# MuMuJun97/semantic_slam_mapping

Hardware: AMD Instinct MI355X
Metric: frames/sec semantic-mapping, 640x480 RGB-D (higher is better)
Workload: dtype u8; 1 GPU; configs[1]: synthetic 640x480 RGB-D + precomputed 12-class masks, 1k frames per GPU, ORB 1000 kp/frame, 5 ref frames, leaf 0.10 m; frames_per_gpu=1000, frames_all_gpus=1000, batch_frames=250, matcher_halo_frames=0, parallelism=single GPU

## Files before the change

semantic_slam_mapping_amd/csrc/kernels_orb.hip:

```cpp
#include "ssm_internal.h"
#include "../../include/ssm/fast_quick_core.h"
#include <cstdlib>
#include <type_traits>
#include <algorithm>
#include <cstring>
#include <vector>

#define WAVE 64

template <bool VEC>
__global__ void gray_kernel(const uint8_t* __restrict__ img, int W, int H, int stride0, uint8_t* __restrict__ pyr, int pyr_bytes)
{
    const int quads = stride0 >> 2;
    const int q = blockIdx.x * blockDim.x + threadIdx.x;
    if (q >= quads * H) return;
    const int y = q / quads, x = (q - y * quads) << 2;
    const uint8_t* src = img + (size_t)blockIdx.y * W * H * 3 + ((size_t)y * W + x) * 3;
    uint8_t* dst = pyr + (size_t)blockIdx.y * pyr_bytes + (size_t)y * stride0 + x;
    uint32_t out = 0;
    if (x >= W) { *reinterpret_cast<uint32_t*>(dst) = 0; return; }
    if (VEC) {
        const uint32_t* s = reinterpret_cast<const uint32_t*>(src);
        uint32_t a = s[0], b = s[1], c = s[2];
        uint32_t p0 = ((a & 255) * 1868 + ((a >> 8) & 255) * 9617 + ((a >> 16) & 255) * 4899 + 8192) >> 14;
// ... 858 lines not shown
    for (int k = 0; k < OT_T / 64; k++) { const uint32_t x = sw[k]; tot += x; if (k < w) base += x; }
    __syncthreads();
    total = tot;
    return inc - v + base;
}
#ifdef SSM_OT_PROF
__device__ unsigned long long ot_prof[8][8];
#define OTP_T0 long long otp_ = clock64();
#define OTP(k) { const long long n_ = clock64(); if (threadIdx.x == 0) atomicAdd(&ot_prof[blockIdx.y & 7][k], (unsigned long long)(n_ - otp_)); otp_ = n_; }
#define OTP_CNT(k) { if (threadIdx.x == 0) atomicAdd(&ot_prof[blockIdx.y & 7][k], 1ull); }
#else
#define OTP_T0
#define OTP(k)
#define OTP_CNT(k)
#endif
template <int NODES>
__global__ void __launch_bounds__(OT_T, NODES == 256 ? 8 : 1)
octree_kernel(OrbGeom g, const cand_t* __restrict__ cand, const int32_t* __restrict__ ncand, const int32_t* __restrict__ cellmax,
              uint16_t* __restrict__ node_of, uint32_t* __restrict__ sel, int32_t* __restrict__ nsel, int32_t* __restrict__ status)
{
    __shared__ QNode    nd[2][NODES];
    __shared__ uint32_t cnt[2][NODES];
    __shared__ uint32_t sq[2][NODES];
    __shared__ __attribute__((aligned(8))) uint32_t cc[NODES][4];
    __shared__ short    newpos[NODES];
    __shared__ __attribute__((aligned(8))) short childpos[NODES][4];
    __shared__ short    order[NODES];
    unsigned long long* best = reinterpret_cast<unsigned long long*>(&cc[0][0]);
    __shared__ uint16_t lnof[OT_KCAP];
    __shared__ uint16_t cumn[NODES];
    __shared__ uint32_t sscan[OT_T / 64];
    __shared__ int sL, sFinish, sMode, sErr, sValid, sFirst;
    const int l = blockIdx.y, f = blockIdx.x, tid = threadIdx.x;
    OTP_T0
    const LevelGeom& L = g.L[l];
    const int N = L.nfeat;
    int nc = ncand[f * g.nlevels + l];
    if (nc > L.cand_cap) { nc = L.cand_cap; if (tid == 0) atomicOr(status, 1); }
    const cand_t* gkeys = cand + (size_t)f * g.cand_total + L.cand_off;
    uint16_t* gnof = node_of + (size_t)f * g.cand_total + L.cand_off;
    const bool in_lds = nc <= OT_KCAP;
    constexpr int KPT = OT_KCAP / OT_T;
    uint32_t kxr[KPT];
#pragma unroll
    for (int u = 0; u < KPT; u++) kxr[u] = 0u;
#define KEY(i) (gkeys[i])
#define KEYX(i) (gkeys[i].x)
#define NOF(i) (in_lds ? lnof[i] : gnof[i])
#define SETNOF(i, v) do { if (in_lds) lnof[i] = (uint16_t)(v); else gnof[i] = (uint16_t)(v); } while (0)
    uint32_t* out = sel + (size_t)f * g.sel_total + L.sel_off;
    if (nc == 0) { if (tid == 0) nsel[f * g.nlevels + l] = 0; return; }
    const int nIni = L.nIni; const float hX = L.hX;
    for (int i = tid; i < nIni; i += OT_T) {
        QNode q; q.x0 = (short)(int)(hX * (float)i); q.y0 = 0; q.x1 = (short)(int)(hX * (float)(i + 1)); q.y1 = (short)(L.maxBY - L.minBY);
        nd[0][i] = q; cnt[0][i] = 0; sq[0][i] = i;
    }
    if (tid == 0) { sErr = 0; sValid = 0; }
    __syncthreads();
    const int32_t* cm = cellmax + (size_t)f * g.cells_total + L.cell_off;
    int nvalid = 0;
    auto init_trip = [&](auto lds_tag, int i0, cand_t (&k)[OT_UN]) {
        constexpr bool in_lds = decltype(lds_tag)::value;
        int cmv[OT_UN];
#pragma unroll
        for (int u = 0; u < OT_UN; u++) { const int i = i0 + u * OT_T; k[u] = i < nc ? KEY(i) : make_uint2(0u, 0u); }
#pragma unroll
// ... 9 lines not shown
            int b = (int)((float)x / hX); b = min(b, nIni - 1);
            SETNOF(i, b); atomicAdd(&cnt[0][b], 1u); nvalid++;
        }
    };
    if (in_lds) {
#pragma unroll
        for (int t = 0; t < KPT / OT_UN; t++) {
            const int i0 = tid + t * OT_UN * OT_T;
            if (i0 < nc) { cand_t k[OT_UN]; init_trip(std::true_type{}, i0, k); for (int u = 0; u < OT_UN; u++) kxr[t * OT_UN + u] = k[u].x; }
        }
    } else {
        for (int i0 = tid; i0 < nc; i0 += OT_UN * OT_T) { cand_t k[OT_UN]; init_trip(std::false_type{}, i0, k); }
    }
    if (nvalid) atomicAdd(&sValid, nvalid);
    __syncthreads();
    if (sValid == 0) { if (tid == 0) nsel[f * g.nlevels + l] = 0; return; }
    if (tid == 0) {
        int pos = 0;
        for (int i = 0; i < nIni; i++) {
            if (cnt[0][i] == 0) { newpos[i] = -1; continue; }
            nd[1][pos] = nd[0][i]; cnt[1][pos] = cnt[0][i]; sq[1][pos] = sq[0][i]; newpos[i] = (short)pos; pos++;
        }
        sL = pos; sFinish = 0; sMode = 0;
    }
    __syncthreads();
    if (in_lds) { for (int i = tid; i < nc; i += OT_T) { const int o = lnof[i]; if (o != DROPPED) lnof[i] = (uint16_t)newpos[o]; } }
    else        { for (int i = tid; i < nc; i += OT_T) { const int o = gnof[i]; if (o != DROPPED) gnof[i] = (uint16_t)newpos[o]; } }
    int cur = 1;
    __syncthreads();
    OTP(0)
    while (!sFinish) {
// ... 205 lines not shown
    if (sErr && tid == 0) atomicOr(status, 2);
    for (int i = tid; i < Lf; i += OT_T) best[i] = 0ull;
    __syncthreads();
    for (int i0 = tid; i0 < nc; i0 += OT_UN * OT_T) {
        int ni[OT_UN]; cand_t k[OT_UN];
#pragma unroll
        for (int u = 0; u < OT_UN; u++) { const int i = i0 + u * OT_T; ni[u] = i < nc ? (in_lds ? (int)lnof[i] : (int)gnof[i]) : DROPPED; k[u] = i < nc ? KEY(i) : make_uint2(0u, 0u); }
#pragma unroll
        for (int u = 0; u < OT_UN; u++) {
            if (ni[u] == DROPPED) continue;
            const unsigned long long v = ((unsigned long long)(k[u].x >> 24) << 56) | ((unsigned long long)(0xFFFFFFFFu - k[u].y) << 24) | (k[u].x & 0xFFFFFFu);
            atomicMax(&best[ni[u]], v);
        }
    }
    __syncthreads();
    for (int i = tid; i < Lf && i < L.sel_cap; i += OT_T) {
        const unsigned long long v = best[i];
        const uint32_t x = (uint32_t)(v & 4095) + L.minBX, y = (uint32_t)((v >> 12) & 4095) + L.minBY, s = (uint32_t)(v >> 56);
        out[i] = x | (y << 12) | (s << 24);
    }
    if (tid == 0) { nsel[f * g.nlevels + l] = min(Lf, L.sel_cap); if (Lf > L.sel_cap) atomicOr(status, 4); }
    OTP(5)
}
#ifdef SSM_OT_PROF
extern "C" void ssm_debug_octree_prof(void)
{
    unsigned long long h[8][8];
    if (hipMemcpyFromSymbol(h, HIP_SYMBOL(ot_prof), sizeof(h)) != hipSuccess) return;
    for (int l = 0; l < 8; l++) fprintf(stderr, "octree level %d: init %llu count-sweep %llu order %llu rebuild %llu relabel %llu best %llu | passes %llu\n", l, h[l][0], h[l][1], h[l][2], h[l][3], h[l][4], h[l][5], h[l][7]);
    for (auto& r_ : h) for (auto& v_ : r_) v_ = 0;
    (void)hipMemcpyToSymbol(HIP_SYMBOL(ot_prof), h, sizeof(h));
}
#endif
hipError_t k_octree(int n, const OrbGeom& g, const cand_t* cand, const int32_t* ncand, const int32_t* cellmax, uint16_t* node_of,
                    uint32_t* sel, int32_t* nsel, int32_t* status, hipStream_t s)
{
    int need = 0;
    for (int l = 0; l < g.nlevels; l++) need = need > g.L[l].nfeat + 3 ? need : g.L[l].nfeat + 3;
    for (int l = 0; l < g.nlevels; l++) need = need > 4 * g.L[l].nIni + 8 ? need : 4 * g.L[l].nIni + 8;
    if (need <= 256 - 8) octree_kernel<256><<<dim3(n, g.nlevels), OT_T, 0, s>>>(g, cand, ncand, cellmax, node_of, sel, nsel, status);
    else if (need <= 512 - 8) octree_kernel<512><<<dim3(n, g.nlevels), OT_T, 0, s>>>(g, cand, ncand, cellmax, node_of, sel, nsel, status);
    else                 octree_kernel<1024><<<dim3(n, g.nlevels), OT_T, 0, s>>>(g, cand, ncand, cellmax, node_of, sel, nsel, status);
    return hipGetLastError();
}

__device__ __forceinline__ float fast_atan2_deg(float y, float x)
{
    const float p1 = 0.9997878412794807f * (float)(180 / 3.14159265358979323846);
    const float p3 = -0.3258083974640975f * (float)(180 / 3.14159265358979323846);
    const float p5 = 0.1555786518463281f * (float)(180 / 3.14159265358979323846);
    const float p7 = -0.04432655554792128f * (float)(180 / 3.14159265358979323846);
    const float ax = fabsf(x), ay = fabsf(y);
    float a, c, c2;
    if (ax >= ay) { c = ay / (ax + (float)2.2204460492503131e-16); c2 = c * c; a = (((p7 * c2 + p5) * c2 + p3) * c2 + p1) * c; }
    else          { c = ax / (ay + (float)2.2204460492503131e-16); c2 = c * c; a = 90.f - (((p7 * c2 + p5) * c2 + p3) * c2 + p1) * c; }
    if (x < 0) a = 180.f - a;
    if (y < 0) a = 360.f - a;
// ... 17 lines not shown
    const double sn = r + r * (r2 * ps);
    double pc = 1.0 / 20922789888000.0;
    pc = pc * r2 - 1.0 / 87178291200.0;
    pc = pc * r2 + 1.0 / 479001600.0;
    pc = pc * r2 - 1.0 / 3628800.0;
    pc = pc * r2 + 1.0 / 40320.0;
    pc = pc * r2 - 1.0 / 720.0;
    pc = pc * r2 + 1.0 / 24.0;
    pc = pc * r2 - 0.5;
    const double cs = 1.0 + r2 * pc;
    double S, C;
    switch (k & 3) { case 0: S = sn; C = cs; break; case 1: S = cs; C = -sn; break; case 2: S = -sn; C = -cs; break; default: S = -cs; C = sn; break; }
    *s = (float)S; *c = (float)C;
}
__device__ __forceinline__ int wave_total(int v) { return __builtin_amdgcn_readlane((int)wave_incl_scan_u32((uint32_t)v), 63); }
struct KpAux { int32_t m10, m01; float sn, cs; };
#define DP_ROWS_O 31
#define DP_QW_O 3
#define DP_ROWS_B 37
#define DP_QW_B 4
__device__ __forceinline__ bool kp_slot(const OrbGeom& g, const int32_t* __restrict__ ns, int slot, int& l, int& oidx)
{
    if (slot >= g.sel_total) return false;
    l = 0;
    while (l + 1 < g.nlevels && slot >= g.L[l+1].sel_off) l++;
    const int i = slot - g.L[l].sel_off;
    if (i >= ns[l]) return false;
    oidx = i;
    for (int k = 0; k < l; k++) oidx += ns[k];
    return true;
}
struct KpRec { uint32_t off; uint32_t stride_level; int32_t oidx; uint32_t pk; };
__global__ void __launch_bounds__(256)
kp_prepare_kernel(OrbGeom g, const uint32_t* __restrict__ sel, const int32_t* __restrict__ nsel, KpRec* __restrict__ recs, int32_t* __restrict__ nkp)
{
    const int f = blockIdx.y, slot = blockIdx.x * 256 + threadIdx.x;
    const int32_t* ns = nsel + f * g.nlevels;
    if (slot == 0) { int t = 0; for (int l = 0; l < g.nlevels; l++) t += ns[l]; nkp[f] = t; }
    if (slot >= g.sel_total) return;
    int l, oidx;
    KpRec r; r.off = 0; r.stride_level = 0; r.oidx = -1; r.pk = 0;
    if (kp_slot(g, ns, slot, l, oidx)) {
        const LevelGeom& L = g.L[l];
        r.pk = sel[(size_t)f * g.sel_total + slot];
        const int x = r.pk & 4095, y = (r.pk >> 12) & 4095;
        r.off = (uint32_t)(L.img_off + y * L.stride + x); r.stride_level = (uint32_t)L.stride | ((uint32_t)l << 16); r.oidx = oidx;
    }
    recs[(size_t)f * g.sel_total + slot] = r;
}
#define OR_KPW 4
__device__ __forceinline__ uint32_t udot4(uint32_t a, uint32_t b, uint32_t acc) { return __builtin_amdgcn_udot4(a, b, acc, false); }
__global__ void __launch_bounds__(256)
orient_kernel(OrbGeom g, unsigned long long umax_pack, const uint8_t* __restrict__ pyr, const KpRec* __restrict__ recs, KpAux* __restrict__ aux, int nframes)
{
    const int lane = threadIdx.x & 63, wv = threadIdx.x >> 6, f = blockIdx.x;
    const int slot0 = (blockIdx.y * 4 + wv) * OR_KPW;
    if (f >= nframes || slot0 >= g.sel_total) return;
    const int r = lane >> 1, left = !(lane & 1);
    const int v = r <= 2 * SSM_HALF_PATCH ? r - SSM_HALF_PATCH : 0;
    const int d = r <= 2 * SSM_HALF_PATCH ? (int)((umax_pack >> (4 * (v < 0 ? -v : v))) & 15ull) : -1;
    uint32_t M[4];
#pragma unroll
    for (int j = 0; j < 4; j++) {
        uint32_t m = 0;
#pragma unroll
        for (int k = 0; k < 4; k++) {
            const int kk = 4 * j + k;
            const bool keep = left ? (kk >= 16 - d && d > 0) : (kk <= d);
            m |= keep ? (0xFFu << (8 * k)) : 0u;
        }
        M[j] = m;
    }
    const int koff = left ? -16 : 0;
    const uint8_t* fr = pyr + (size_t)f * g.pyr_bytes;
    uint4 px[OR_KPW]; bool ok[OR_KPW]; KpRec rec[OR_KPW];
#pragma unroll
    for (int q = 0; q < OR_KPW; q++) rec[q] = recs[(size_t)f * g.sel_total + min(slot0 + q, g.sel_total - 1)];
#pragma unroll
    for (int q = 0; q < OR_KPW; q++) {
        ok[q] = slot0 + q < g.sel_total && rec[q].oidx >= 0;
        const uint8_t* p = ok[q] ? fr + rec[q].off + v * (int)(rec[q].stride_level & 0xFFFFu) + koff : fr;
        uint4 t; __builtin_memcpy(&t, p, 16);
        px[q] = t;
    }
#pragma unroll
    for (int q = 0; q < OR_KPW; q++) {
        if (!ok[q]) continue;
        const uint32_t a0 = px[q].x & M[0], a1 = px[q].y & M[1], a2 = px[q].z & M[2], a3 = px[q].w & M[3];
        uint32_t si = udot4(a0, 0x01010101u, 0u); si = udot4(a1, 0x01010101u, si); si = udot4(a2, 0x01010101u, si); si = udot4(a3, 0x01010101u, si);
        uint32_t sk = udot4(a0, 0x03020100u, 0u); sk = udot4(a1, 0x07060504u, sk); sk = udot4(a2, 0x0B0A0908u, sk); sk = udot4(a3, 0x0F0E0D0Cu, sk);
        const int sui = (int)sk - (left ? 16 * (int)si : 0);
        const int m10 = wave_total(sui), m01 = wave_total(v * (int)si);
        if (lane == 0) { KpAux a; a.m10 = m10; a.m01 = m01; a.sn = 0.f; a.cs = 0.f; aux[(size_t)f * g.sel_total + slot0 + q] = a; }
    }
}
__global__ void __launch_bounds__(256)
angle_kernel(OrbGeom g, const KpRec* __restrict__ recs, const uint16_t* __restrict__ depth, ssm_camera cam,
             KpAux* __restrict__ aux, ssm_keypoint* __restrict__ kps, float* __restrict__ pos3d)
{
    const int f = blockIdx.y, slot = blockIdx.x * 256 + threadIdx.x;
    if (slot >= g.sel_total) return;
    const KpRec rec = recs[(size_t)f * g.sel_total + slot];
    if (rec.oidx < 0) return;
    const int l = (int)(rec.stride_level >> 16), oidx = rec.oidx;
    const LevelGeom& L = g.L[l];
    const uint32_t pk = rec.pk;
    const int x = pk & 4095, y = (pk >> 12) & 4095, score = pk >> 24;
    KpAux a = aux[(size_t)f * g.sel_total + slot];
    const float angle = fast_atan2_deg((float)a.m01, (float)a.m10);
    contract_sincos(angle * (float)(3.14159265358979323846 / 180.f), &a.sn, &a.cs);
    aux[(size_t)f * g.sel_total + slot] = a;
    ssm_keypoint kp;
    kp.x = (float)x; kp.y = (float)y;
    if (l != 0) { kp.x *= L.sf; kp.y *= L.sf; }
    kp.size = (float)SSM_PATCH * L.sf; kp.angle = angle; kp.response = (float)score; kp.octave = l; kp.class_id = -1;
    kps[(size_t)f * g.cap + oidx] = kp;
    if (pos3d) {
        float px = 0.f, py = 0.f, pz = 0.f;
        if (depth) {
            const int u = (int)kp.x, v = (int)kp.y;
            const uint16_t d = depth[(size_t)f * g.W * g.H + (size_t)v * g.W + u];
            if (d != 0) {
                pz = (float)((double)d / cam.scale);
                px = (float)(((double)u - cam.cx) * (double)pz / cam.fx);
                py = (float)(((double)v - cam.cy) * (double)pz / cam.fy);
            }
        }
        float* o = pos3d + ((size_t)f * g.cap + oidx) * 3;
        o[0] = px; o[1] = py; o[2] = pz;
    }
}
#define ROW_SHL(v, n) ((uint32_t)__builtin_amdgcn_update_dpp(0, (int)(v), 0x100 + (n), 0xF, 0xF, true))
#define BR_KPW 2
#define BR_NIT 4
#define BR_PW ((DP_ROWS_B * DP_QW_B + 63) / 64)
__global__ void __launch_bounds__(256)
brief_kernel(OrbGeom g, const uint8_t* __restrict__ blur, const KpRec* __restrict__ recs,
             const float* __restrict__ pattern_f, const KpAux* __restrict__ aux, uint8_t* __restrict__ desc, int nframes)
{
    __shared__ uint4 pb[4][BR_KPW][DP_ROWS_B * DP_QW_B];
    const int lane = threadIdx.x & 63, wv = __builtin_amdgcn_readfirstlane(threadIdx.x >> 6), f = blockIdx.x;
    const int slot0 = (blockIdx.y * 4 + wv) * (BR_KPW * BR_NIT);
    if (f >= nframes || slot0 >= g.sel_total) return;
    const KpRec* rp = recs + (size_t)f * g.sel_total;
    const KpAux* ap = aux + (size_t)f * g.sel_total;
    typedef float f2 __attribute__((ext_vector_type(2)));
    const float4* pf = reinterpret_cast<const float4*>(pattern_f) + lane * 4;
    const float4 pq[4] = {pf[0], pf[1], pf[2], pf[3]};
    uint4 pw[BR_KPW][BR_PW];
    KpRec rec[BR_KPW], nrec[BR_KPW];
    auto load_recs = [&](int it, KpRec (&r)[BR_KPW]) {
#pragma unroll
        for (int j = 0; j < BR_KPW; j++) {
            const int slot = slot0 + it * BR_KPW + j;
            r[j].oidx = -1;
            if (it < BR_NIT && slot < g.sel_total) r[j] = rp[slot];
        }
    };
    auto fetch = [&](const KpRec (&r)[BR_KPW]) {
#pragma unroll
        for (int j = 0; j < BR_KPW; j++) {
            if (r[j].oidx < 0) continue;
            const int stride = (int)(r[j].stride_level & 0xFFFFu), x = r[j].pk & 4095, y = (r[j].pk >> 12) & 4095;
            const uint8_t* lv = blur + (size_t)f * g.blur_bytes;
            const int boff = g.L[r[j].stride_level >> 16].boff;
            const int xb0 = (x - 18) & ~15;
#pragma unroll
            for (int q = 0; q < BR_PW; q++) {
                const int e = lane + 64 * q, rr = e >> 2, c = e & 3, gx = xb0 + 16 * c;
                pw[j][q] = (e < DP_ROWS_B * DP_QW_B && gx < stride) ? *reinterpret_cast<const uint4*>(lv + blur_off(boff, stride, gx, y + rr - 18)) : make_uint4(0, 0, 0, 0);
            }
        }
    };
    load_recs(0, rec);
    fetch(rec);
    for (int it = 0; it < BR_NIT; it++) {
        load_recs(it + 1, nrec);
        KpAux a[BR_KPW];
#pragma unroll
        for (int j = 0; j < BR_KPW; j++) if (rec[j].oidx >= 0) a[j] = ap[slot0 + it * BR_KPW + j];
        __builtin_amdgcn_wave_barrier();
#pragma unroll
        for (int j = 0; j < BR_KPW; j++) {
            if (rec[j].oidx < 0) continue;
#pragma unroll
            for (int q = 0; q < BR_PW; q++) { const int e = lane + 64 * q; if (e < DP_ROWS_B * DP_QW_B) pb[wv][j][e] = pw[j][q]; }
        }
        fetch(nrec);
        __builtin_amdgcn_wave_barrier();
#pragma unroll
        for (int j = 0; j < BR_KPW; j++) {
            if (rec[j].oidx < 0) continue;
            const int x = rec[j].pk & 4095, xb0 = (x - 18) & ~15;
            const uint8_t* bb = reinterpret_cast<const uint8_t*>(pb[wv][j]) + 18 * (DP_QW_B * 16) + (x - xb0);
            const float sb = a[j].sn, ca = a[j].cs;
            const f2 s2 = {sb, sb}, c2 = {ca, ca}, magic = {12582912.0f, 12582912.0f};
            uint32_t nib = 0;
#pragma unroll
            for (int k = 0; k < 4; k++) {
                const f2 X = {pq[k].x, pq[k].z}, Y = {pq[k].y, pq[k].w};
                const f2 xs = X * s2, yc = Y * c2, xc = X * c2, ys = Y * s2;
                const f2 yy = (xs + yc) + magic, xx = (xc - ys) + magic;
                const uint32_t i0 = (__float_as_uint(yy.x) << 6) + __float_as_uint(xx.x) - 0x4B400000u * 65u;
                const uint32_t i1 = (__float_as_uint(yy.y) << 6) + __float_as_uint(xx.y) - 0x4B400000u * 65u;
                const int t0 = bb[(int)i0], t1 = bb[(int)i1];
                nib |= (uint32_t)(t0 < t1) << k;
            }
            uint32_t b = nib | (ROW_SHL(nib, 1) << 4);
            b |= ROW_SHL(b, 2) << 8;
            b |= ROW_SHL(b, 4) << 16;
            const uint32_t hi = ROW_SHL(b, 8);
            if ((lane & 15) == 0)
                reinterpret_cast<uint2*>(desc + ((size_t)f * g.cap + rec[j].oidx) * 32)[lane >> 4] = make_uint2(b, hi);
        }
#pragma unroll
        for (int j = 0; j < BR_KPW; j++) rec[j] = nrec[j];
    }
}
hipError_t k_describe(int n, const OrbGeom& g, const uint8_t* pyr, const uint8_t* blur, const uint32_t* sel,
                      const int32_t* nsel, const float* pattern_f, const uint16_t* depth, ssm_camera cam, void* kpaux,
                      ssm_keypoint* kps, uint8_t* desc, float* pos3d, int32_t* nkp, hipStream_t s)
{
    unsigned long long um = 0;
    for (int v = 0; v <= SSM_HALF_PATCH; v++) um |= (unsigned long long)(g.umax[v] & 15) << (4 * v);
    KpAux* aux = reinterpret_cast<KpAux*>(kpaux);
    KpRec* recs = reinterpret_cast<KpRec*>(aux + (size_t)n * g.sel_total);
    kp_prepare_kernel<<<dim3((g.sel_total + 255) / 256, n), 256, 0, s>>>(g, sel, nsel, recs, nkp);
    orient_kernel<<<dim3((n + 7) & ~7, (g.sel_total + 4 * OR_KPW - 1) / (4 * OR_KPW)), 256, 0, s>>>(g, um, pyr, recs, aux, n);
    angle_kernel<<<dim3((g.sel_total + 255) / 256, n), 256, 0, s>>>(g, recs, depth, cam, aux, kps, pos3d);
    brief_kernel<<<dim3((n + 7) & ~7, (g.sel_total + 4 * BR_KPW * BR_NIT - 1) / (4 * BR_KPW * BR_NIT)), 256, 0, s>>>(g, blur, recs, pattern_f, aux, desc, n);
    return hipGetLastError();
}
```

semantic_slam_mapping_amd/csrc/ssm_abi.hip:

```cpp
#include "ssm_ctx.h"
#include "ssm_host.h"
#include <set>

static const int8_t k_default_pattern[1024] = {
#include "orb_pattern.inc"
};
thread_local std::string g_create_err;
int host_fail(ssm_ctx* c, int code, const std::string& msg) { if (c) c->err = msg; else g_create_err = msg; return code; }
std::unique_lock<std::mutex> host_lock(ssm_ctx* c) { return c ? std::unique_lock<std::mutex>(c->mu) : std::unique_lock<std::mutex>(); }

int ensure_scratch(ssm_ctx* c, size_t bytes, DevBuf<uint8_t>* buf)
{
    DevBuf<uint8_t>& b = buf ? *buf : c->d_scratch;
    if (bytes <= b.bytes()) return SSM_OK;
    if (b) hipStreamSynchronize(c->main.stream);
    return b.alloc(c, bytes);
}
int ensure_pinned(ssm_ctx* c, size_t bytes)
{
    if (bytes <= c->h_pinned.bytes()) return SSM_OK;
    if (c->h_pinned) hipStreamSynchronize(c->main.stream);
    if (c->h_pinned.alloc(c, bytes)) FAIL(c, SSM_E_HIP, "hipHostMalloc failed");
    return SSM_OK;
}
// ... 50 lines not shown
    c->knn_match_ratio = 0.8; c->tracker_ref_frames = 5;
    c->mapper_resolution = 0.1; c->mapper_max_distance = 40;
    c->camera.cx = 318.6; c->camera.cy = 255.3; c->camera.fx = 517.3; c->camera.fy = 516.5; c->camera.scale = 1000.0;
    c->max_batch = 16; c->voxel_capacity_log2 = 20; c->brief_pattern = nullptr;
    c->voxel_max_capacity_log2 = 28; c->sgbm_form = 0; c->sgbm_streams = 0; c->stereo_batch = 0;
}
extern "C" const char* ssm_version(void) { return "ssm_hip 0.1 (gfx950)"; }
extern "C" const char* ssm_last_error(const ssm_ctx* c) { return c ? c->err.c_str() : g_create_err.c_str(); }

static int orb_work_alloc(ssm_ctx* c, OrbWork& w)
{
    const OrbGeom& g = c->g; const int B = c->B;
    DALLOC(c, w.pyr, (size_t)B * g.pyr_bytes + 16); DALLOC(c, w.blur, (size_t)B * g.blur_bytes);
    DALLOC(c, w.ncand, k_fast_ncand_pad(B, g) + k_fast_cellmax_ints(B, g)); w.cellmax = w.ncand + k_fast_ncand_pad(B, g);
    DALLOC(c, w.cand, (size_t)B * g.cand_total); DALLOC(c, w.nodeof, (size_t)B * g.cand_total);
    DALLOC(c, w.sel, (size_t)B * g.sel_total); DALLOC(c, w.nsel, (size_t)B * g.nlevels);
    DALLOC(c, w.kpaux, (size_t)B * g.sel_total * 2);
    return SSM_OK;
}
template <class T> static int upload(ssm_ctx* c, DevBuf<T>& d, const std::vector<T>& v)
{
    DALLOC(c, d, v.size());
    HIPCHK(c, hipMemcpy(d, v.data(), v.size() * sizeof(T), hipMemcpyHostToDevice));
    return SSM_OK;
}
#define UPLOAD(ctx, buf, vec) do { int r__ = upload(ctx, buf, vec); if (r__) return r__; } while (0)
static int ctx_init(ssm_ctx* c)
{
    const ssm_config& cfg = c->cfg; const OrbPlan& P = c->plan; const OrbGeom& g = c->g; const int B = c->B, W = g.W, H = g.H;
    HIPCHK(c, c->main.stream.ensure());
    c->dev.id = c->device;
// ... 139 lines not shown
{
    const OrbGeom& g = c->g;
    if (plan.bands) {
        prof_begin(c, s, "pyramid"); HIPCHK(c, k_pyramid_bands(d_img, channels, nb, g, w.pyr, plan, c->pyr_tabs.yofs, c->pyr_tabs.ya, c->pyr_tabs.xgrp, c->pyr_tabs.xgrp8, s)); prof_end(c, s);
        return SSM_OK;
    }
    prof_begin(c, s, "gray");      HIPCHK(c, k_gray(d_img, channels, nb, g, w.pyr, s)); prof_end(c, s);
    prof_begin(c, s, "pyramid");   HIPCHK(c, k_pyramid(nb, g, w.pyr, c->pyr_tabs.xofs, c->pyr_tabs.xa, c->pyr_tabs.yofs, c->pyr_tabs.ya, c->pyr_tabs.xgrp, s)); prof_end(c, s);
    return SSM_OK;
}
static int orb_detect(ssm_ctx* c, hipStream_t s, OrbWork& w, const uint8_t* d_img, int channels, int nb)
{
    const OrbGeom& g = c->g;
    { const int r = make_pyramid(c, s, w, d_img, channels, nb, nb > 1 ? c->pyr_bands : c->pyr_bands1); if (r) return r; }
    prof_begin(c, s, "fast");      HIPCHK(c, k_fast(nb, g, w.pyr, w.cand, w.ncand, w.cellmax, s)); prof_end(c, s);
    prof_begin(c, s, "octree");    HIPCHK(c, k_octree(nb, g, w.cand, w.ncand, w.cellmax, w.nodeof, w.sel, w.nsel, c->d_status, s)); prof_end(c, s);
    prof_begin(c, s, "blur");      HIPCHK(c, c->blur_mfma ? k_blur_mfma(nb, g, w.pyr, w.blur, c->d_blur_tab, s) : k_blur(nb, g, w.pyr, w.blur, s)); prof_end(c, s);
    return SSM_OK;
}
static int orb_describe(ssm_ctx* c, hipStream_t s, OrbWork& w, const uint16_t* d_depth, int nb, ssm_keypoint* kps, uint8_t* desc, float* pos3d, int32_t* nkp)
{
    prof_begin(c, s, "describe");  HIPCHK(c, k_describe(nb, c->g, w.pyr, w.blur, w.sel, w.nsel, c->d_pattern_f, d_depth, c->cfg.camera, w.kpaux, kps, desc, pos3d, nkp, s)); prof_end(c, s);
    return SSM_OK;
}
static int run_orb(ssm_ctx* c, hipStream_t s, OrbWork& w, const uint8_t* d_img, int channels, const uint16_t* d_depth, int nb,
                   ssm_keypoint* kps, uint8_t* desc, float* pos3d, int32_t* nkp)
{
    const int r = orb_detect(c, s, w, d_img, channels, nb);
    return r ? r : orb_describe(c, s, w, d_depth, nb, kps, desc, pos3d, nkp);
}

extern "C" void ssm_debug_live_allocations(int* buffers, size_t* device_bytes, size_t* pinned_bytes)
{
    if (buffers) *buffers = DevBufLive::buffers.load();
    if (device_bytes) *device_bytes = DevBufLive::device_bytes.load();
    if (pinned_bytes) *pinned_bytes = DevBufLive::pinned_bytes.load();
}
// ... 556 lines not shown
```

semantic_slam_mapping_amd/csrc/ssm_ctx.h:

```cpp
#pragma once
#include "ssm_internal.h"
#include "pnp_chain.h"
#include "ssm_map_plan.h"
#include <rccl/rccl.h>
#include <cmath>
#include <cfloat>
#include <cstring>
#include <cstdlib>
#include <atomic>
#include <memory>
#include <mutex>
#include <type_traits>
#include <utility>
#include <functional>
#include <string>
#include <vector>
#define SSM_HIDDEN __attribute__((visibility("hidden")))

struct DevBufLive { static inline std::atomic<int> buffers{0}; static inline std::atomic<size_t> device_bytes{0}, pinned_bytes{0}; };
template <class T, bool Pinned = false> class DevBuf {
    T* p = nullptr; size_t nbytes = 0;
public:
    DevBuf() = default;
    DevBuf(const DevBuf&) = delete; DevBuf& operator=(const DevBuf&) = delete;
// ... 113 lines not shown
};
struct SegNetState {
    bool set[SEG_LAYERS] = {};
    DevBuf<void> w[SEG_LAYERS]; DevBuf<float> scale[SEG_LAYERS], shift[SEG_LAYERS];
    DevBuf<void> ww[SEG_LAYERS];
    int cinp[SEG_LAYERS], coutp[SEG_LAYERS], coutstore[SEG_LAYERS];
    int batch = 0;
    DevBuf<void> actA, actB; void* last_logits = nullptr ; DevBuf<uint8_t> code[5], labels;
    DevBuf<int32_t> pre_xofs, pre_yofs, post_xofs, post_yofs;
    DevBuf<int16_t> pre_xa, pre_ya, post_xa, post_ya;
    DevBuf<uint8_t> d_sem_gen;
};

struct OrbWork {
    DevBuf<uint8_t> pyr, blur; DevBuf<int32_t> ncand; int32_t* cellmax = nullptr ; DevBuf<cand_t> cand; DevBuf<uint16_t> nodeof;
    DevBuf<uint32_t> sel; DevBuf<int32_t> nsel; DevBuf<uint4> kpaux;
};
struct MfWork {
    int cap_n = 0, n = 0, w = 0, h = 0; size_t cap_px = 0;
    DevBuf<uint8_t> always, cand, filled; DevBuf<int32_t> labels, area, overlap, info; PinBuf<int32_t> h_info;
    DevBuf<uint8_t> in_sem, in_motion, out_mask;
};
struct ssm_cloud { ssm_point* d = nullptr; int n = 0; int device = 0; int slab = -1; DevBuf<uint8_t> run; };
struct ssm_carve_view { DevBuf<uint16_t> depth; int w = 0, h = 0, device = 0; ssm_camera cam{}; };
struct ssm_render_target {
    int w = 0, h = 0, device = 0; bool rendered = false;
    DevBuf<unsigned long long> keys; DevBuf<uint16_t> depth; DevBuf<uint8_t> bgr, label; DevBuf<int32_t> index;
    DevBuf<uint16_t> f_depth; DevBuf<uint8_t> f_sem, cls;
};
struct RenderWork { DevBuf<int32_t> info; PinBuf<int32_t> h_info; DevBuf<unsigned long long> counts; PinBuf<unsigned long long> h_counts; };
struct ssm_align_view { DevBuf<uint16_t> depth; DevBuf<uint8_t> normals; int w = 0, h = 0, device = 0; ssm_camera cam{}; double tol_abs = 0; int32_t tol_rel_ppm = 0; };
// ... 120 lines not shown
```

semantic_slam_mapping_amd/csrc/ssm_internal.h:

```cpp
#pragma once
#include <hip/hip_runtime.h>
#include <stdint.h>
#include <vector>
#include "../../include/ssm_hip.h"
#include "ssm_orb_plan.h"
#include "cloud_table.h"

#define SSM_VOX_EMPTY ((int64_t)-1)
inline size_t up256(size_t v) { return (v + 255) & ~(size_t)255; }
struct Carve {
    size_t off = 0; template <class T> size_t take(size_t count, size_t align = 256) { const size_t at = (off + align - 1) & ~(align - 1); off = at + count * sizeof(T); return at; }
    size_t end() { return take<uint8_t>(0); }
};

typedef uint2 cand_t;

struct DeviceInfo { int id = 0, cus = 256, max_lds = 160 * 1024; };
hipError_t allow_dynamic_lds(const void* fn, size_t bytes, int limit);

hipError_t k_gray(const uint8_t* img, int channels, int n, const OrbGeom& g, uint8_t* pyr, hipStream_t s);
hipError_t k_copy_gray_strided(const uint8_t* img, int stride, const OrbGeom& g, uint8_t* pyr, hipStream_t s);
hipError_t k_pyramid(int n, const OrbGeom& g, uint8_t* pyr, const int32_t* const* xofs, const int16_t* const* xa,
                     const int32_t* const* yofs, const int16_t* const* ya, const void* const* xgroups, hipStream_t s);
hipError_t k_pyramid_bands(const uint8_t* img, int channels, int n, const OrbGeom& g, uint8_t* pyr, const PyrBandPlan& p,
                           const int32_t* const* yofs, const int16_t* const* ya, const void* const* xgroups, const void* const* xgroups8, hipStream_t s);
hipError_t k_blur(int n, const OrbGeom& g, const uint8_t* pyr, uint8_t* blur, hipStream_t s);
hipError_t k_blur_mfma(int n, const OrbGeom& g, const uint8_t* pyr, uint8_t* blur, const void* tab, hipStream_t s);
hipError_t k_fast(int n, const OrbGeom& g, const uint8_t* pyr, cand_t* cand, int32_t* ncand, int32_t* cellmax , hipStream_t s);
size_t k_fast_ncand_pad(int nframes, const OrbGeom& g);
size_t k_fast_cellmax_ints(int nframes, const OrbGeom& g);
hipError_t k_octree(int n, const OrbGeom& g, const cand_t* cand, const int32_t* ncand, const int32_t* cellmax, uint16_t* node_of,
                    uint32_t* sel, int32_t* nsel, int32_t* status, hipStream_t s);
hipError_t k_describe(int n, const OrbGeom& g, const uint8_t* pyr, const uint8_t* blur, const uint32_t* sel,
                      const int32_t* nsel, const float* pattern_f , const uint16_t* depth, ssm_camera cam, void* kpaux ,
                      ssm_keypoint* kps, uint8_t* desc, float* pos3d, int32_t* nkp, hipStream_t s);

struct MatchPair { int32_t qoff, nq, toff, nt, out_slot; };
hipError_t k_match_pairs(const uint8_t* desc, const MatchPair* pairs, int npairs, double ratio, int cap,
                         ssm_dmatch* out, int32_t* nout, int32_t* knn_idx, int32_t* knn_dist, hipStream_t s);
hipError_t k_match_seq(const uint8_t* desc, const int32_t* nkp, int f0, int n, int R, int hist, double ratio, int cap,
                       ssm_dmatch* out, int32_t* nout, int32_t* pend , hipStream_t s);

#define SSM_MATCH_DESC_BYTES 128
hipError_t k_match_expand(const uint8_t* desc, const int32_t* nkp, int row0, int nrows, int cap, int capT, uint8_t* eq, uint8_t* et, hipStream_t s);
hipError_t k_match_seq_mfma(const uint8_t* eq, const uint8_t* et, const int32_t* nkp, int f0, int n, int R, int hist, double ratio, int cap, int capT,
                            void* knn , ssm_dmatch* out, int32_t* nout, hipStream_t s);

hipError_t k_moving_mask(const uint8_t* sem, int n, int w, int h, uint8_t* mask, hipStream_t s);
// ... 158 lines not shown
```

Baseline: 190,700 frames/s.

## Emit keypoint records from octree and fuse angle into orient kernel

The octree kernel now writes full KpRec records (image offset, stride/level, per-level index, packed key) directly and pads unused slots, which removes the separate kp_prepare kernel and the intermediate sel buffer. The angle/keypoint/3D-position work is folded into orient_kernel through a shared-memory handoff of moments. Output indices are rebuilt from per-level bases with a wave scan in orient and brief. The goal is two fewer launches and less global traffic per batch, at the cost of writing every sel_cap slot in octree and some extra per-block scan work.

```diff
diff --git a/semantic_slam_mapping_amd/csrc/kernels_orb.hip b/semantic_slam_mapping_amd/csrc/kernels_orb.hip
--- a/semantic_slam_mapping_amd/csrc/kernels_orb.hip
+++ b/semantic_slam_mapping_amd/csrc/kernels_orb.hip
@@ -896,10 +896,13 @@
 #define OTP(k)
 #define OTP_CNT(k)
 #endif
+struct KpRec { uint32_t off; uint32_t stride_level; int32_t idx; uint32_t pk; };
+struct KpAux { int32_t m10, m01; float sn, cs; };
+static inline KpRec* kp_recs(void* kpaux, int n, const OrbGeom& g) { return reinterpret_cast<KpRec*>(reinterpret_cast<KpAux*>(kpaux) + (size_t)n * g.sel_total); }
 template <int NODES>
 __global__ void __launch_bounds__(OT_T, NODES == 256 ? 8 : 1)
 octree_kernel(OrbGeom g, const cand_t* __restrict__ cand, const int32_t* __restrict__ ncand, const int32_t* __restrict__ cellmax,
-              uint16_t* __restrict__ node_of, uint32_t* __restrict__ sel, int32_t* __restrict__ nsel, int32_t* __restrict__ status)
+              uint16_t* __restrict__ node_of, KpRec* __restrict__ recs, int32_t* __restrict__ nsel, int32_t* __restrict__ status)
 {
     __shared__ QNode    nd[2][NODES];
     __shared__ uint32_t cnt[2][NODES];
@@ -930,8 +933,9 @@
 #define KEYX(i) (gkeys[i].x)
 #define NOF(i) (in_lds ? lnof[i] : gnof[i])
 #define SETNOF(i, v) do { if (in_lds) lnof[i] = (uint16_t)(v); else gnof[i] = (uint16_t)(v); } while (0)
-    uint32_t* out = sel + (size_t)f * g.sel_total + L.sel_off;
-    if (nc == 0) { if (tid == 0) nsel[f * g.nlevels + l] = 0; return; }
+    KpRec* out = recs + (size_t)f * g.sel_total + L.sel_off;
+    const KpRec none = {0u, 0u, -1, 0u};
+    if (nc == 0) { for (int i = tid; i < L.sel_cap; i += OT_T) out[i] = none; if (tid == 0) nsel[f * g.nlevels + l] = 0; return; }
     const int nIni = L.nIni; const float hX = L.hX;
     for (int i = tid; i < nIni; i += OT_T) {
         QNode q; q.x0 = (short)(int)(hX * (float)i); q.y0 = 0; q.x1 = (short)(int)(hX * (float)(i + 1)); q.y1 = (short)(L.maxBY - L.minBY);
@@ -971,7 +975,7 @@
     }
     if (nvalid) atomicAdd(&sValid, nvalid);
     __syncthreads();
-    if (sValid == 0) { if (tid == 0) nsel[f * g.nlevels + l] = 0; return; }
+    if (sValid == 0) { for (int i = tid; i < L.sel_cap; i += OT_T) out[i] = none; if (tid == 0) nsel[f * g.nlevels + l] = 0; return; }
     if (tid == 0) {
         int pos = 0;
         for (int i = 0; i < nIni; i++) {
@@ -1207,10 +1211,14 @@
         }
     }
     __syncthreads();
-    for (int i = tid; i < Lf && i < L.sel_cap; i += OT_T) {
-        const unsigned long long v = best[i];
-        const uint32_t x = (uint32_t)(v & 4095) + L.minBX, y = (uint32_t)((v >> 12) & 4095) + L.minBY, s = (uint32_t)(v >> 56);
-        out[i] = x | (y << 12) | (s << 24);
+    for (int i = tid; i < L.sel_cap; i += OT_T) {
+        KpRec r = none;
+        if (i < Lf) {
+            const unsigned long long v = best[i];
+            const uint32_t x = (uint32_t)(v & 4095) + L.minBX, y = (uint32_t)((v >> 12) & 4095) + L.minBY, s = (uint32_t)(v >> 56);
+            r.off = (uint32_t)L.img_off + y * (uint32_t)L.stride + x; r.stride_level = (uint32_t)L.stride | ((uint32_t)l << 16); r.idx = i; r.pk = x | (y << 12) | (s << 24);
+        }
+        out[i] = r;
     }
     if (tid == 0) { nsel[f * g.nlevels + l] = min(Lf, L.sel_cap); if (Lf > L.sel_cap) atomicOr(status, 4); }
     OTP(5)
@@ -1226,14 +1234,15 @@
 }
 #endif
 hipError_t k_octree(int n, const OrbGeom& g, const cand_t* cand, const int32_t* ncand, const int32_t* cellmax, uint16_t* node_of,
-                    uint32_t* sel, int32_t* nsel, int32_t* status, hipStream_t s)
-{
+                    void* kpaux, int32_t* nsel, int32_t* status, hipStream_t s)
+{
+    KpRec* recs = kp_recs(kpaux, n, g);
     int need = 0;
     for (int l = 0; l < g.nlevels; l++) need = need > g.L[l].nfeat + 3 ? need : g.L[l].nfeat + 3;
     for (int l = 0; l < g.nlevels; l++) need = need > 4 * g.L[l].nIni + 8 ? need : 4 * g.L[l].nIni + 8;
-    if (need <= 256 - 8) octree_kernel<256><<<dim3(n, g.nlevels), OT_T, 0, s>>>(g, cand, ncand, cellmax, node_of, sel, nsel, status);
-    else if (need <= 512 - 8) octree_kernel<512><<<dim3(n, g.nlevels), OT_T, 0, s>>>(g, cand, ncand, cellmax, node_of, sel, nsel, status);
-    else                 octree_kernel<1024><<<dim3(n, g.nlevels), OT_T, 0, s>>>(g, cand, ncand, cellmax, node_of, sel, nsel, status);
+    if (need <= 256 - 8) octree_kernel<256><<<dim3(n, g.nlevels), OT_T, 0, s>>>(g, cand, ncand, cellmax, node_of, recs, nsel, status);
+    else if (need <= 512 - 8) octree_kernel<512><<<dim3(n, g.nlevels), OT_T, 0, s>>>(g, cand, ncand, cellmax, node_of, recs, nsel, status);
+    else                 octree_kernel<1024><<<dim3(n, g.nlevels), OT_T, 0, s>>>(g, cand, ncand, cellmax, node_of, recs, nsel, status);
     return hipGetLastError();
 }
 
@@ -1281,48 +1290,36 @@
     *s = (float)S; *c = (float)C;
 }
 __device__ __forceinline__ int wave_total(int v) { return __builtin_amdgcn_readlane((int)wave_incl_scan_u32((uint32_t)v), 63); }
-struct KpAux { int32_t m10, m01; float sn, cs; };
 #define DP_ROWS_O 31
 #define DP_QW_O 3
 #define DP_ROWS_B 37
 #define DP_QW_B 4
-__device__ __forceinline__ bool kp_slot(const OrbGeom& g, const int32_t* __restrict__ ns, int slot, int& l, int& oidx)
-{
-    if (slot >= g.sel_total) return false;
-    l = 0;
-    while (l + 1 < g.nlevels && slot >= g.L[l+1].sel_off) l++;
-    const int i = slot - g.L[l].sel_off;
-    if (i >= ns[l]) return false;
-    oidx = i;
-    for (int k = 0; k < l; k++) oidx += ns[k];
-    return true;
-}
-struct KpRec { uint32_t off; uint32_t stride_level; int32_t oidx; uint32_t pk; };
-__global__ void __launch_bounds__(256)
-kp_prepare_kernel(OrbGeom g, const uint32_t* __restrict__ sel, const int32_t* __restrict__ nsel, KpRec* __restrict__ recs, int32_t* __restrict__ nkp)
-{
-    const int f = blockIdx.y, slot = blockIdx.x * 256 + threadIdx.x;
-    const int32_t* ns = nsel + f * g.nlevels;
-    if (slot == 0) { int t = 0; for (int l = 0; l < g.nlevels; l++) t += ns[l]; nkp[f] = t; }
-    if (slot >= g.sel_total) return;
-    int l, oidx;
-    KpRec r; r.off = 0; r.stride_level = 0; r.oidx = -1; r.pk = 0;
-    if (kp_slot(g, ns, slot, l, oidx)) {
-        const LevelGeom& L = g.L[l];
-        r.pk = sel[(size_t)f * g.sel_total + slot];
-        const int x = r.pk & 4095, y = (r.pk >> 12) & 4095;
-        r.off = (uint32_t)(L.img_off + y * L.stride + x); r.stride_level = (uint32_t)L.stride | ((uint32_t)l << 16); r.oidx = oidx;
-    }
-    recs[(size_t)f * g.sel_total + slot] = r;
+__device__ __forceinline__ int level_bases(const OrbGeom& g, const int32_t* __restrict__ ns, int lane, int& total)
+{
+    const int c = lane < g.nlevels ? ns[lane] : 0;
+    const int inc = (int)wave_incl_scan_u32((uint32_t)c);
+    total = __builtin_amdgcn_readlane(inc, 63);
+    return inc - c;
 }
 #define OR_KPW 4
 __device__ __forceinline__ uint32_t udot4(uint32_t a, uint32_t b, uint32_t acc) { return __builtin_amdgcn_udot4(a, b, acc, false); }
 __global__ void __launch_bounds__(256)
-orient_kernel(OrbGeom g, unsigned long long umax_pack, const uint8_t* __restrict__ pyr, const KpRec* __restrict__ recs, KpAux* __restrict__ aux, int nframes)
-{
+orient_kernel(OrbGeom g, unsigned long long umax_pack, const uint8_t* __restrict__ pyr, const KpRec* __restrict__ recs, const int32_t* __restrict__ nsel,
+              const uint16_t* __restrict__ depth, ssm_camera cam, KpAux* __restrict__ aux, ssm_keypoint* __restrict__ kps, float* __restrict__ pos3d, int32_t* __restrict__ nkp, int nframes)
+{
+    __shared__ int2 mom[4 * OR_KPW];
     const int lane = threadIdx.x & 63, wv = threadIdx.x >> 6, f = blockIdx.x;
     const int slot0 = (blockIdx.y * 4 + wv) * OR_KPW;
-    if (f >= nframes || slot0 >= g.sel_total) return;
+    if (f >= nframes) return;
+    KpRec mine = {0u, 0u, -1, 0u}; int base = 0;
+    if (wv == 0) {
+        const int slot = blockIdx.y * 4 * OR_KPW + lane;
+        if (lane < 4 * OR_KPW && slot < g.sel_total) mine = recs[(size_t)f * g.sel_total + slot];
+        int total;
+        const int bases = level_bases(g, nsel + f * g.nlevels, lane, total);
+        if (blockIdx.y == 0 && lane == 0) nkp[f] = total;
+        base = __shfl(bases, (int)(mine.stride_level >> 16), 64);
+    }
     const int r = lane >> 1, left = !(lane & 1);
     const int v = r <= 2 * SSM_HALF_PATCH ? r - SSM_HALF_PATCH : 0;
     const int d = r <= 2 * SSM_HALF_PATCH ? (int)((umax_pack >> (4 * (v < 0 ? -v : v))) & 15ull) : -1;
@@ -1345,7 +1342,7 @@
     for (int q = 0; q < OR_KPW; q++) rec[q] = recs[(size_t)f * g.sel_total + min(slot0 + q, g.sel_total - 1)];
 #pragma unroll
     for (int q = 0; q < OR_KPW; q++) {
-        ok[q] = slot0 + q < g.sel_total && rec[q].oidx >= 0;
+        ok[q] = slot0 + q < g.sel_total && rec[q].idx >= 0;
         const uint8_t* p = ok[q] ? fr + rec[q].off + v * (int)(rec[q].stride_level & 0xFFFFu) + koff : fr;
         uint4 t; __builtin_memcpy(&t, p, 16);
         px[q] = t;
@@ -1358,43 +1355,37 @@
         uint32_t sk = udot4(a0, 0x03020100u, 0u); sk = udot4(a1, 0x07060504u, sk); sk = udot4(a2, 0x0B0A0908u, sk); sk = udot4(a3, 0x0F0E0D0Cu, sk);
         const int sui = (int)sk - (left ? 16 * (int)si : 0);
         const int m10 = wave_total(sui), m01 = wave_total(v * (int)si);
-        if (lane == 0) { KpAux a; a.m10 = m10; a.m01 = m01; a.sn = 0.f; a.cs = 0.f; aux[(size_t)f * g.sel_total + slot0 + q] = a; }
-    }
-}
-__global__ void __launch_bounds__(256)
-angle_kernel(OrbGeom g, const KpRec* __restrict__ recs, const uint16_t* __restrict__ depth, ssm_camera cam,
-             KpAux* __restrict__ aux, ssm_keypoint* __restrict__ kps, float* __restrict__ pos3d)
-{
-    const int f = blockIdx.y, slot = blockIdx.x * 256 + threadIdx.x;
-    if (slot >= g.sel_total) return;
-    const KpRec rec = recs[(size_t)f * g.sel_total + slot];
-    if (rec.oidx < 0) return;
-    const int l = (int)(rec.stride_level >> 16), oidx = rec.oidx;
+        if (lane == 0) mom[wv * OR_KPW + q] = make_int2(m10, m01);
+    }
+    __syncthreads();
+    if (mine.idx < 0) return;
+    const int2 mq = mom[lane];
+    const int l = (int)(mine.stride_level >> 16), oidx = base + mine.idx;
     const LevelGeom& L = g.L[l];
-    const uint32_t pk = rec.pk;
+    const uint32_t pk = mine.pk;
     const int x = pk & 4095, y = (pk >> 12) & 4095, score = pk >> 24;
-    KpAux a = aux[(size_t)f * g.sel_total + slot];
+    KpAux a; a.m10 = mq.x; a.m01 = mq.y;
     const float angle = fast_atan2_deg((float)a.m01, (float)a.m10);
     contract_sincos(angle * (float)(3.14159265358979323846 / 180.f), &a.sn, &a.cs);
-    aux[(size_t)f * g.sel_total + slot] = a;
+    aux[(size_t)f * g.sel_total + blockIdx.y * 4 * OR_KPW + lane] = a;
     ssm_keypoint kp;
     kp.x = (float)x; kp.y = (float)y;
     if (l != 0) { kp.x *= L.sf; kp.y *= L.sf; }
     kp.size = (float)SSM_PATCH * L.sf; kp.angle = angle; kp.response = (float)score; kp.octave = l; kp.class_id = -1;
     kps[(size_t)f * g.cap + oidx] = kp;
     if (pos3d) {
-        float px = 0.f, py = 0.f, pz = 0.f;
+        float px3 = 0.f, py3 = 0.f, pz3 = 0.f;
         if (depth) {
-            const int u = (int)kp.x, v = (int)kp.y;
-            const uint16_t d = depth[(size_t)f * g.W * g.H + (size_t)v * g.W + u];
-            if (d != 0) {
-                pz = (float)((double)d / cam.scale);
-                px = (float)(((double)u - cam.cx) * (double)pz / cam.fx);
-                py = (float)(((double)v - cam.cy) * (double)pz / cam.fy);
+            const int u = (int)kp.x, w = (int)kp.y;
+            const uint16_t dz = depth[(size_t)f * g.W * g.H + (size_t)w * g.W + u];
+            if (dz != 0) {
+                pz3 = (float)((double)dz / cam.scale);
+                px3 = (float)(((double)u - cam.cx) * (double)pz3 / cam.fx);
+                py3 = (float)(((double)w - cam.cy) * (double)pz3 / cam.fy);
             }
         }
         float* o = pos3d + ((size_t)f * g.cap + oidx) * 3;
-        o[0] = px; o[1] = py; o[2] = pz;
+        o[0] = px3; o[1] = py3; o[2] = pz3;
     }
 }
 #define ROW_SHL(v, n) ((uint32_t)__builtin_amdgcn_update_dpp(0, (int)(v), 0x100 + (n), 0xF, 0xF, true))
@@ -1402,7 +1393,7 @@
 #define BR_NIT 4
 #define BR_PW ((DP_ROWS_B * DP_QW_B + 63) / 64)
 __global__ void __launch_bounds__(256)
-brief_kernel(OrbGeom g, const uint8_t* __restrict__ blur, const KpRec* __restrict__ recs,
+brief_kernel(OrbGeom g, const uint8_t* __restrict__ blur, const KpRec* __restrict__ recs, const int32_t* __restrict__ nsel,
              const float* __restrict__ pattern_f, const KpAux* __restrict__ aux, uint8_t* __restrict__ desc, int nframes)
 {
     __shared__ uint4 pb[4][BR_KPW][DP_ROWS_B * DP_QW_B];
@@ -1420,14 +1411,14 @@
 #pragma unroll
         for (int j = 0; j < BR_KPW; j++) {
             const int slot = slot0 + it * BR_KPW + j;
-            r[j].oidx = -1;
+            r[j].idx = -1;
             if (it < BR_NIT && slot < g.sel_total) r[j] = rp[slot];
         }
     };
     auto fetch = [&](const KpRec (&r)[BR_KPW]) {
 #pragma unroll
         for (int j = 0; j < BR_KPW; j++) {
-            if (r[j].oidx < 0) continue;
+            if (r[j].idx < 0) continue;
             const int stride = (int)(r[j].stride_level & 0xFFFFu), x = r[j].pk & 4095, y = (r[j].pk >> 12) & 4095;
             const uint8_t* lv = blur + (size_t)f * g.blur_bytes;
             const int boff = g.L[r[j].stride_level >> 16].boff;
@@ -1440,16 +1431,18 @@
         }
     };
     load_recs(0, rec);
+    int total;
+    const int bases = level_bases(g, nsel + f * g.nlevels, lane, total);
     fetch(rec);
     for (int it = 0; it < BR_NIT; it++) {
         load_recs(it + 1, nrec);
         KpAux a[BR_KPW];
 #pragma unroll
-        for (int j = 0; j < BR_KPW; j++) if (rec[j].oidx >= 0) a[j] = ap[slot0 + it * BR_KPW + j];
+        for (int j = 0; j < BR_KPW; j++) if (rec[j].idx >= 0) a[j] = ap[slot0 + it * BR_KPW + j];
         __builtin_amdgcn_wave_barrier();
 #pragma unroll
         for (int j = 0; j < BR_KPW; j++) {
-            if (rec[j].oidx < 0) continue;
+            if (rec[j].idx < 0) continue;
 #pragma unroll
             for (int q = 0; q < BR_PW; q++) { const int e = lane + 64 * q; if (e < DP_ROWS_B * DP_QW_B) pb[wv][j][e] = pw[j][q]; }
         }
@@ -1457,7 +1450,7 @@
         __builtin_amdgcn_wave_barrier();
 #pragma unroll
         for (int j = 0; j < BR_KPW; j++) {
-            if (rec[j].oidx < 0) continue;
+            if (rec[j].idx < 0) continue;
             const int x = rec[j].pk & 4095, xb0 = (x - 18) & ~15;
             const uint8_t* bb = reinterpret_cast<const uint8_t*>(pb[wv][j]) + 18 * (DP_QW_B * 16) + (x - xb0);
             const float sb = a[j].sn, ca = a[j].cs;
@@ -1477,24 +1470,23 @@
             b |= ROW_SHL(b, 2) << 8;
             b |= ROW_SHL(b, 4) << 16;
             const uint32_t hi = ROW_SHL(b, 8);
+            const int oidx = __builtin_amdgcn_readlane(bases, __builtin_amdgcn_readfirstlane((int)(rec[j].stride_level >> 16))) + rec[j].idx;
             if ((lane & 15) == 0)
-                reinterpret_cast<uint2*>(desc + ((size_t)f * g.cap + rec[j].oidx) * 32)[lane >> 4] = make_uint2(b, hi);
+                reinterpret_cast<uint2*>(desc + ((size_t)f * g.cap + oidx) * 32)[lane >> 4] = make_uint2(b, hi);
         }
 #pragma unroll
         for (int j = 0; j < BR_KPW; j++) rec[j] = nrec[j];
     }
 }
-hipError_t k_describe(int n, const OrbGeom& g, const uint8_t* pyr, const uint8_t* blur, const uint32_t* sel,
+hipError_t k_describe(int n, const OrbGeom& g, const uint8_t* pyr, const uint8_t* blur,
                       const int32_t* nsel, const float* pattern_f, const uint16_t* depth, ssm_camera cam, void* kpaux,
                       ssm_keypoint* kps, uint8_t* desc, float* pos3d, int32_t* nkp, hipStream_t s)
 {
     unsigned long long um = 0;
     for (int v = 0; v <= SSM_HALF_PATCH; v++) um |= (unsigned long long)(g.umax[v] & 15) << (4 * v);
     KpAux* aux = reinterpret_cast<KpAux*>(kpaux);
-    KpRec* recs = reinterpret_cast<KpRec*>(aux + (size_t)n * g.sel_total);
-    kp_prepare_kernel<<<dim3((g.sel_total + 255) / 256, n), 256, 0, s>>>(g, sel, nsel, recs, nkp);
-    orient_kernel<<<dim3((n + 7) & ~7, (g.sel_total + 4 * OR_KPW - 1) / (4 * OR_KPW)), 256, 0, s>>>(g, um, pyr, recs, aux, n);
-    angle_kernel<<<dim3((g.sel_total + 255) / 256, n), 256, 0, s>>>(g, recs, depth, cam, aux, kps, pos3d);
-    brief_kernel<<<dim3((n + 7) & ~7, (g.sel_total + 4 * BR_KPW * BR_NIT - 1) / (4 * BR_KPW * BR_NIT)), 256, 0, s>>>(g, blur, recs, pattern_f, aux, desc, n);
+    const KpRec* recs = kp_recs(kpaux, n, g);
+    orient_kernel<<<dim3((n + 7) & ~7, (g.sel_total + 4 * OR_KPW - 1) / (4 * OR_KPW)), 256, 0, s>>>(g, um, pyr, recs, nsel, depth, cam, aux, kps, pos3d, nkp, n);
+    brief_kernel<<<dim3((n + 7) & ~7, (g.sel_total + 4 * BR_KPW * BR_NIT - 1) / (4 * BR_KPW * BR_NIT)), 256, 0, s>>>(g, blur, recs, nsel, pattern_f, aux, desc, n);
     return hipGetLastError();
 }
diff --git a/semantic_slam_mapping_amd/csrc/ssm_abi.hip b/semantic_slam_mapping_amd/csrc/ssm_abi.hip
--- a/semantic_slam_mapping_amd/csrc/ssm_abi.hip
+++ b/semantic_slam_mapping_amd/csrc/ssm_abi.hip
@@ -88,7 +88,7 @@
     DALLOC(c, w.pyr, (size_t)B * g.pyr_bytes + 16); DALLOC(c, w.blur, (size_t)B * g.blur_bytes);
     DALLOC(c, w.ncand, k_fast_ncand_pad(B, g) + k_fast_cellmax_ints(B, g)); w.cellmax = w.ncand + k_fast_ncand_pad(B, g);
     DALLOC(c, w.cand, (size_t)B * g.cand_total); DALLOC(c, w.nodeof, (size_t)B * g.cand_total);
-    DALLOC(c, w.sel, (size_t)B * g.sel_total); DALLOC(c, w.nsel, (size_t)B * g.nlevels);
+    DALLOC(c, w.nsel, (size_t)B * g.nlevels);
     DALLOC(c, w.kpaux, (size_t)B * g.sel_total * 2);
     return SSM_OK;
 }
@@ -258,13 +258,13 @@
     const OrbGeom& g = c->g;
     { const int r = make_pyramid(c, s, w, d_img, channels, nb, nb > 1 ? c->pyr_bands : c->pyr_bands1); if (r) return r; }
     prof_begin(c, s, "fast");      HIPCHK(c, k_fast(nb, g, w.pyr, w.cand, w.ncand, w.cellmax, s)); prof_end(c, s);
-    prof_begin(c, s, "octree");    HIPCHK(c, k_octree(nb, g, w.cand, w.ncand, w.cellmax, w.nodeof, w.sel, w.nsel, c->d_status, s)); prof_end(c, s);
+    prof_begin(c, s, "octree");    HIPCHK(c, k_octree(nb, g, w.cand, w.ncand, w.cellmax, w.nodeof, w.kpaux, w.nsel, c->d_status, s)); prof_end(c, s);
     prof_begin(c, s, "blur");      HIPCHK(c, c->blur_mfma ? k_blur_mfma(nb, g, w.pyr, w.blur, c->d_blur_tab, s) : k_blur(nb, g, w.pyr, w.blur, s)); prof_end(c, s);
     return SSM_OK;
 }
 static int orb_describe(ssm_ctx* c, hipStream_t s, OrbWork& w, const uint16_t* d_depth, int nb, ssm_keypoint* kps, uint8_t* desc, float* pos3d, int32_t* nkp)
 {
-    prof_begin(c, s, "describe");  HIPCHK(c, k_describe(nb, c->g, w.pyr, w.blur, w.sel, w.nsel, c->d_pattern_f, d_depth, c->cfg.camera, w.kpaux, kps, desc, pos3d, nkp, s)); prof_end(c, s);
+    prof_begin(c, s, "describe");  HIPCHK(c, k_describe(nb, c->g, w.pyr, w.blur, w.nsel, c->d_pattern_f, d_depth, c->cfg.camera, w.kpaux, kps, desc, pos3d, nkp, s)); prof_end(c, s);
     return SSM_OK;
 }
 static int run_orb(ssm_ctx* c, hipStream_t s, OrbWork& w, const uint8_t* d_img, int channels, const uint16_t* d_depth, int nb,
diff --git a/semantic_slam_mapping_amd/csrc/ssm_ctx.h b/semantic_slam_mapping_amd/csrc/ssm_ctx.h
--- a/semantic_slam_mapping_amd/csrc/ssm_ctx.h
+++ b/semantic_slam_mapping_amd/csrc/ssm_ctx.h
@@ -151,7 +151,7 @@
 
 struct OrbWork {
     DevBuf<uint8_t> pyr, blur; DevBuf<int32_t> ncand; int32_t* cellmax = nullptr ; DevBuf<cand_t> cand; DevBuf<uint16_t> nodeof;
-    DevBuf<uint32_t> sel; DevBuf<int32_t> nsel; DevBuf<uint4> kpaux;
+    DevBuf<int32_t> nsel; DevBuf<uint4> kpaux;
 };
 struct MfWork {
     int cap_n = 0, n = 0, w = 0, h = 0; size_t cap_px = 0;
diff --git a/semantic_slam_mapping_amd/csrc/ssm_internal.h b/semantic_slam_mapping_amd/csrc/ssm_internal.h
--- a/semantic_slam_mapping_amd/csrc/ssm_internal.h
+++ b/semantic_slam_mapping_amd/csrc/ssm_internal.h
@@ -30,8 +30,8 @@
 size_t k_fast_ncand_pad(int nframes, const OrbGeom& g);
 size_t k_fast_cellmax_ints(int nframes, const OrbGeom& g);
 hipError_t k_octree(int n, const OrbGeom& g, const cand_t* cand, const int32_t* ncand, const int32_t* cellmax, uint16_t* node_of,
-                    uint32_t* sel, int32_t* nsel, int32_t* status, hipStream_t s);
-hipError_t k_describe(int n, const OrbGeom& g, const uint8_t* pyr, const uint8_t* blur, const uint32_t* sel,
+                    void* kpaux , int32_t* nsel, int32_t* status, hipStream_t s);
+hipError_t k_describe(int n, const OrbGeom& g, const uint8_t* pyr, const uint8_t* blur,
                       const int32_t* nsel, const float* pattern_f , const uint16_t* depth, ssm_camera cam, void* kpaux ,
                       ssm_keypoint* kps, uint8_t* desc, float* pos3d, int32_t* nkp, hipStream_t s);
 
```

After: 188,400 frames/s. 0.988x the previous value.
